# sgl-project/rbg

Hardware: NVIDIA B200
Metric: replica_x_node_affinity_scores_per_sec (higher is better)
Workload: dtype f32

## Files before the change

rbg_b200/csrc/kernels.cuh:

```cuda
#pragma once
#include <cuda_runtime.h>
#include <stdint.h>

#include "../../include/rbgtopo.h"

namespace rbgtopo {

constexpr int KS = RBGTOPO_MAX_STEP_REPLICAS;
constexpr int MAXP = RBGTOPO_MAX_STEP_ROLES;
constexpr int MAXQ = RBGTOPO_MAX_GROUP_ROLES;
constexpr int SCORE_THREADS = 256;
constexpr int SCORE_WARPS = SCORE_THREADS / 32;
constexpr int BASE_THREADS = 256;
constexpr int BASE_TILE_ROWS = 256;
constexpr int BASE_TILE_NNZ = 6144;
constexpr int FMIN_SMEM_MAX = 131072;
constexpr uint32_t FULL = 0xFFFFFFFFu;

struct TopoDev {
  int n;
  int slab_lo, slab_hi;
  int slab_stride;
  const int* row_ptr;
  const int* col;
// ... 23 lines not shown
  const int* perm;
  unsigned long long* lists;
  const unsigned long long* lists_all;
  long long part_stride;
  unsigned long long* merged;
  unsigned long long* excl;
  const unsigned long long* excl_all;
  long long excl_part_stride;
  int* dstar;
  int* assign;
  int* status;
  int* domain_out;
  int* corr;
  int* corr_cnt;
  int corr_w;
};

constexpr int EMIT_TAB_WORDS = 12;
__host__ __device__ __forceinline__ int emit_pack_role(int count, int demand, int need, int flags) {
  return count | (need << 6) | ((flags & RBGTOPO_ROLE_EXCLUSIVE) << 11) | (demand << 12);
}

__host__ __device__ __forceinline__ int emit_pack_row(int demand, int need, bool rexcl) {
  return need | ((rexcl ? 1 : 0) << 5) | (demand << 6);
}

__device__ __forceinline__ uint32_t orderable_u32(float x) {
  uint32_t b = __float_as_uint(x);
  return b ^ ((b >> 31) ? 0xFFFFFFFFu : 0x80000000u);
}
// ... 257 lines not shown
```

rbg_b200/csrc/plan_group.cuh:

```cuda
#pragma once
#include "select_fast.cuh"

namespace rbgtopo {

struct GroupTab {
  int* node;
  int* cons;
  float* aw;
  int mask, HT;
  int* cnt;
  int* dSlot;
  float* dBase;
  int* dFree;
  int* dAvail;
  int* dDom;
};
struct GroupRole {
  int count, demand, need, flags;
};

__host__ __device__ inline size_t group_smem_bytes(int QB, int PB, int HT, int CAP) {
  return (size_t)HT * 4 * (2 + QB) + (size_t)CAP * 20 +
         (size_t)PB * KS * (3 * 8 + 3 * 4) +
         (size_t)MAXP * 16 + (size_t)MAXP * RBGTOPO_MAX_GROUP_ROLES * 4;
// ... 215 lines not shown
      const bool rexcl = excl && (sR[wi][4 * ri + 3] & RBGTOPO_ROLE_EXCLUSIVE);
      sRec[wi][lane] = emit_pack_row(sR[wi][4 * ri + 2], max(0, min(need, RBGTOPO_NEED_CAP)), rexcl);
    }
    __syncwarp();
    for (int p = 0; p < P; ++p) {
      const int cnt = sCount[wi][p];
      const int2 rr = make_int2(sRec[wi][p], gid);
      if (lane < cnt && row + lane < n_rows) rtab[row + lane] = rr;
      row += cnt;
    }
    if (lane < P) sPl[wi][sRole[wi][lane]] += sCount[wi][lane];
    __syncwarp();
  }
}

template <bool DIRECT>
__global__ void __launch_bounds__(32 * MAXP, 4) k_plan_group(TopoDev t, BatchDev b, int QB, int HT, int CAP, int record) {
  extern __shared__ __align__(16) unsigned char pg_smem[];
  __shared__ int sTakenNode[KS], sTakenAmt[KS], sTakenRole[KS], sRowB[KS], sRowN[KS];
  __shared__ int sDstar, sCnt, sNew, sStatus, sAny, sCorrN;
  const int tid = threadIdx.x, warp = tid >> 5, lane = tid & 31, nthreads = blockDim.x, nwarps = nthreads >> 5;
  const int PB = nwarps;
  GroupTab T;
  T.node = reinterpret_cast<int*>(pg_smem);
  T.cons = T.node + HT;
  T.aw = reinterpret_cast<float*>(T.cons + HT);
  T.mask = HT - 1;
  T.HT = HT;
  T.cnt = &sCnt;
  T.dSlot = reinterpret_cast<int*>(T.aw + (size_t)QB * HT);
// ... 11 lines not shown
  float* sPair = reinterpret_cast<float*>(sRole + MAXP);

  if (record) pdl_launch_dependents();
  PCLK(30);
#ifdef RBGTOPO_PHASE_CLOCKS
  if (tid == 0 && blockIdx.x < 2048) { g_cta_ns[blockIdx.x * 4] = pg_gtime(); g_cta_ns[blockIdx.x * 4 + 3] = pg_smid(); }
#endif
  int wave_i = 0;
  int step = b.perm ? b.perm[blockIdx.x] : blockIdx.x;
  __shared__ int sGR[DIRECT ? 4 * RBGTOPO_MAX_GROUP_ROLES : 1];
  __shared__ int sGP[DIRECT ? RBGTOPO_MAX_GROUP_ROLES * RBGTOPO_MAX_GROUP_ROLES : 1];
  __shared__ int sPlaced[DIRECT ? RBGTOPO_MAX_GROUP_ROLES : 1];
  __shared__ int sWRole[DIRECT ? RBGTOPO_MAX_STEP_ROLES : 1], sWCount[DIRECT ? RBGTOPO_MAX_STEP_ROLES : 1];
  __shared__ int sWP, sWN, sCr, sTk;
  int g_rep0 = 0, g_pend = 0, g_i0 = 0, g_stat = 0, g_dom = -1;
  StepHdr h;
  if (DIRECT) {
    const int* rec = b.blob + RBGTOPO_HDR_WORDS + (size_t)step * RBGTOPO_GROUP_WORDS;
    h.gid = rec[0];
    h.flags = rec[1] & (RBGTOPO_STEP_EXCLUSIVE | RBGTOPO_STEP_GANG);
    h.fixed_domain = (rec[1] & RBGTOPO_STEP_EXCLUSIVE) ? rec[2] : -1;
    h.Q = rec[3];
    h.role_off = rec[4];
    h.pair_off = rec[5];
    h.n_anchors = rec[6];
    h.anchor_off = rec[7];
    h.i0 = 0;
    g_rep0 = rec[8];
    g_pend = rec[9];
    h.P = 0; h.R = 0; h.rep_off = g_rep0; h.rolerow_off = 0; h.next_step = 0; h.n_cons = 0; h.cons_off = 0;
  } else {
    h = load_hdr(b, step);
  }
  for (int i = tid; i < HT; i += nthreads) {
    T.node[i] = -1;
    T.cons[i] = 0;
  }
  for (int i = tid; i < QB * HT; i += nthreads) T.aw[i] = 0.0f;
  if (tid == 0) sCnt = 0;
  if (DIRECT) {
    for (int i = tid; i < 4 * h.Q; i += nthreads) sGR[i] = b.blob[h.role_off + i];
    for (int i = tid; i < h.Q * h.Q; i += nthreads) sGP[i] = b.blob[h.pair_off + i];
    if (tid < RBGTOPO_MAX_GROUP_ROLES) sPlaced[tid] = 0;
    if (tid == 0) { sCr = 0; sTk = 0; }
  }
  const bool excl_step = (h.flags & RBGTOPO_STEP_EXCLUSIVE) != 0;
  const bool gang = (h.flags & RBGTOPO_STEP_GANG) != 0;
  const int gid = h.gid, Q = h.Q;
  int fixed = excl_step ? h.fixed_domain : -1;
  g_dom = fixed;
  const size_t stride = (size_t)t.slab_stride;
  __syncthreads();

  {
    const int* anc = b.blob + h.anchor_off;
    for (int a = warp; a < h.n_anchors - h.i0; a += nwarps) gtab_add_anchor(t, T, anc[3 * a], anc[3 * a + 1], anc[3 * a + 2], 0);
  }
  int n_new = 0;
  int cnt_done = 0;

  while (true) {
    PCLK(wave_i * 8 + 0);
    const unsigned long long ob0 = lane < t.n ? t.order_all[lane] : 0ull;
    if (DIRECT) {
      if (tid == 0) {
        int cr = sCr, tk = sTk;
        const int P = wave_next(sGR, Q, cr, tk, sWRole, sWCount);
// ... 305 lines not shown
```

rbg_b200/csrc/rbgtopo.cu:

```cuda
#include <cuda_runtime.h>
#include <cub/device/device_radix_sort.cuh>
#include <nvtx3/nvToolsExt.h>

#include <algorithm>
#include <chrono>
#include <climits>
#include <cstdarg>
#include <cstdio>
#include <cstdlib>
#include <cstring>
#include <functional>
#include <memory>
#include <map>
#include <mutex>
#include <shared_mutex>
#include <string>
#include <vector>

#include "kernels.cuh"
#include "plan.cuh"
#include "score.cuh"
#include "emit_tma.cuh"
#include "emit_rows.cuh"
#include "select.cuh"
// ... 119 lines not shown
  long long patch_cap = 0;
  int max_cap = 0;
  std::vector<int> poff;
};

struct Batch {
  bool in_use = false;
  bool staged = false;
  bool ran = false;
  bool early_emit = false;
  bool d2h_enqueued = false;
  uint64_t epoch = 0;
  cudaStream_t stream = nullptr;
  cudaStream_t stream2 = nullptr;
  cudaEvent_t ev[8] = {};
  std::vector<cudaEvent_t> it_ev;
  int passes = 0, pend_launches = 0, untimed_or_timed_passes = 0;
  bool shard_timed = false;
  BatchMeta m;
  DevBuf<int> blob;
  DevBuf<float> matrix;
  DevBuf<unsigned long long> lists, merged, excl;
  DevBuf<int> cand;
  DevBuf<long long> emit_clk;
  DevBuf<int> etab, emit_ctr;
  DevBuf<int2> rtab;
  bool any_excl = false;
  int perm_n = 0;
  std::vector<char> pass_mid;
  const int32_t* prestaged_h = nullptr;
// ... 2 lines not shown
  bool tev = false;
  DevBuf<int> corr, corr_cnt;
  std::vector<int> wave_begin, wave_maxp;
  std::vector<int> step_group;
  std::vector<int> step_row;
  DevBuf<int> gsrc;
  long long aux_off = -1;
  int g_lo = 0;
  std::vector<int> grp_flags, grp_assign_off, grp_pending, grp_fixed;
  DevBuf<int> out;
  PinBuf<int> h_in, h_out;
  ~Batch() {
    if (stream) cudaStreamDestroy(stream);
    if (stream2) cudaStreamDestroy(stream2);
    for (auto& e : ev) if (e) cudaEventDestroy(e);
    for (auto& e : it_ev) cudaEventDestroy(e);
  }
};

}

struct rbgtopo_ctx {
  rbgtopo_config cfg{};
  int sm_count = 148;
  int slab_lo = 0, slab_hi = 0, slab_stride = 0, lc = 1, chunk = 2048;
  std::shared_mutex topo_mu;
  uint64_t topo_epoch = 0;
  std::mutex pool_mu;
  Topology topo;
  std::vector<std::unique_ptr<Batch>> batches;
  cudaStream_t ext_stream = nullptr;
  bool use_ext_stream = false;
  std::atomic<bool> kernel_timing{false};
  cudaStream_t topo_stream = nullptr;
  cudaEvent_t base_ready = nullptr;
  cudaEvent_t topo_ready = nullptr, ev_base_a = nullptr, ev_base_b = nullptr, fence_ev = nullptr;
  bool base_timing_pending = false;
  PinBuf<int> h_free[2], h_owner[2];
  cudaEvent_t stage_ev[2] = {nullptr, nullptr};
  unsigned stage_idx = 0;
  std::mutex stat_mu;
  DevBuf<unsigned long long> xbuf;
  DevBuf<int> p2p_ctr;
  P2PDev p2p{};
  int p2p_rows_cap = 0;
  bool p2p_ready = false;
  unsigned long long p2p_seq = 0;
  long long p2p_bytes_last = 0;
  std::vector<void*> p2p_opened;
  rbgtopo_timing last{};
  std::vector<float> last_score_ms, last_select_ms;
// ... 31 lines not shown
                          : (kEmitNoRegCap ? k_emit_tma<2, 1, false> : k_emit_tma<2, 4, false>);
}
const int kEmitBlockSteps =
    getenv("RBGTOPO_EMIT_BLOCK") ? std::min(EMIT_MAX_BLOCK, std::max(1, atoi(getenv("RBGTOPO_EMIT_BLOCK")))) : 4;
const int kSplitMinGroups =
    getenv("RBGTOPO_SPLIT_MIN_GROUPS") ? std::max(2, atoi(getenv("RBGTOPO_SPLIT_MIN_GROUPS"))) : (1 << 30);
const bool kCompactSortKey = getenv("RBGTOPO_WIDE_SORT_KEY") == nullptr;
const bool kRefreshGraph = getenv("RBGTOPO_NO_REFRESH_GRAPH") == nullptr;
const bool kSmallSort = getenv("RBGTOPO_SMALL_SORT") != nullptr;
const bool kVerifyPlan = getenv("RBGTOPO_VERIFY_PLAN") != nullptr;
const int kHostThreads = getenv("RBGTOPO_HOST_THREADS") ? std::max(1, atoi(getenv("RBGTOPO_HOST_THREADS"))) : 4;
const int kHostParallelMinGroups = getenv("RBGTOPO_HOST_PARALLEL_MIN") ? std::max(1, atoi(getenv("RBGTOPO_HOST_PARALLEL_MIN"))) : 4096;

inline bool timing_events(const rbgtopo_ctx* c) { return kProfileHost || c->kernel_timing.load(std::memory_order_relaxed); }

void compute_slab(rbgtopo_ctx* c, int n) {
  const int W = c->cfg.world, r = c->cfg.rank;
  auto bound = [&](int g) -> int {
    if (g <= 0) return 0;
    if (g >= W) return n;
    long long b = (long long)g * n / W;
    return (int)(b / 128 * 128);
  };
  c->slab_lo = bound(r);
  c->slab_hi = bound(r + 1);
  int max_len = 0;
  for (int g = 0; g < W; ++g) max_len = std::max(max_len, bound(g + 1) - bound(g));
  int tcfg = c->cfg.chunk_nodes > 0 ? c->cfg.chunk_nodes : 2048;
  tcfg = std::min(2048, std::max(128, round_up(tcfg, 128)));
  c->lc = std::max(1, (max_len + tcfg - 1) / tcfg);
// ... 95 lines not shown
  }
  return RBGTOPO_OK;
}

int enqueue_refresh(rbgtopo_ctx* c, cudaStream_t s, int part) {
  Topology& T = c->topo;
  if (part & 1) {
  k_prep<<<(T.n + 255) / 256, 256, 0, s>>>(T.n, T.free_.p, T.domain.p, T.owner.p, T.fmin.p,
                                           T.node_owner.p);
  const int fmin_bytes = round_up(T.n, 16);
  const int staged = T.n <= FMIN_SMEM_MAX ? 1 : 0;
  const size_t smem = (size_t)2 * (BASE_TILE_NNZ + 8) * 4 + (staged ? fmin_bytes : 0);
  const TopoDev td = topo_dev(c);
  k_base<<<T.n_tiles, BASE_THREADS, smem, s>>>(td, T.tiles.p, staged, fmin_bytes, T.base.p);
  }
  if (part == 3) CK(cudaEventRecord(c->base_ready, s));
  if (!(part & 2)) {
    CK(cudaGetLastError());
    return RBGTOPO_OK;
  }
  const TopoDev td = topo_dev(c);
  const int slab_len = c->slab_hi - c->slab_lo;
  auto p2_bytes = [](int n) { int p2 = 32; while (p2 < n) p2 <<= 1; return (size_t)p2 * 8; };
  if (slab_len > 0 && slab_len <= ORDER_SMALL_MAX && kSmallSort) {
    k_order_sort_small<<<1, ORDER_SMALL_THREADS, p2_bytes(slab_len), s>>>(T.base.p, c->slab_lo, c->slab_hi, T.order.p);
  } else if (slab_len > 0) {
    k_order_keys<<<(slab_len + 255) / 256, 256, 0, s>>>(td, c->slab_lo, c->slab_hi, T.key_nb, T.okeys.p);
    size_t tmp_bytes = T.sort_tmp.cap;
    CK(cub::DeviceRadixSort::SortKeysDescending(T.sort_tmp.p, tmp_bytes, T.okeys.p, T.order.p, slab_len, 0, T.key_bits, s));
    if (T.key_nb) k_order_expand<<<(slab_len + 255) / 256, 256, 0, s>>>(T.order.p, slab_len, T.key_nb);
  }
// ... 31 lines not shown
      if (g) cudaGraphDestroy(g);
      (void)cudaGetLastError();
    };
    capture(1, &T.refresh_exec);
    if (T.refresh_exec) capture(2, &T.order_exec);
    if (!T.order_exec && T.refresh_exec) {
      cudaGraphExecDestroy(T.refresh_exec);
      T.refresh_exec = nullptr;
    }
    T.refresh_ready = true;
  }
  const bool tev = timing_events(c);
  if (tev) CK(cudaEventRecord(c->ev_base_a, s));
  if (T.refresh_exec) {
    CK(cudaGraphLaunch(T.refresh_exec, s));
    CK(cudaEventRecord(c->base_ready, s));
    CK(cudaGraphLaunch(T.order_exec, s));
  } else {
    int rc = enqueue_refresh(c, s, 3);
    if (rc) return rc;
  }
  if (tev) CK(cudaEventRecord(c->ev_base_b, s));
  CK(cudaEventRecord(c->topo_ready, s));
  T.pos_valid = c->cfg.world == 1;
  c->base_timing_pending = tev;
  CK(cudaGetLastError());
  if (sync) {
    CK(cudaStreamSynchronize(s));
    harvest_base_ms(c);
  }
  std::lock_guard<std::mutex> g(c->stat_mu);
  c->launches += 3;
  return RBGTOPO_OK;
}

inline long long emit_items(int ns, int lc) {
  return (long long)((ns + kEmitBlockSteps - 1) / kEmitBlockSteps) * lc * kEmitBlockSteps;
}
// ... 107 lines not shown
  std::lock_guard<std::mutex> g(c->pool_mu);
  for (auto& b : c->batches)
    if (!b->in_use) {
      b->in_use = true;
      *out = b.get();
      return RBGTOPO_OK;
    }
  auto nb = std::make_unique<Batch>();
  CK(cudaStreamCreateWithFlags(&nb->stream, cudaStreamNonBlocking));
  {
    int lo = 0, hi = 0;
    CK(cudaDeviceGetStreamPriorityRange(&lo, &hi));
    CK(cudaStreamCreateWithPriority(&nb->stream2, cudaStreamNonBlocking, kSelectHighPriority ? hi : lo));
  }
  for (auto& e : nb->ev) CK(cudaEventCreate(&e));
  nb->in_use = true;
  *out = nb.get();
  c->batches.push_back(std::move(nb));
  return RBGTOPO_OK;
}
void release_batch(rbgtopo_ctx* c, Batch* b) {
  std::lock_guard<std::mutex> g(c->pool_mu);
  b->wave_begin.clear();
  b->d2h_enqueued = false;
  b->in_use = false;
  b->staged = false;
  b->ran = false;
}

cudaStream_t stream_of(rbgtopo_ctx* c, Batch* b) { return c->use_ext_stream ? c->ext_stream : b->stream; }
// ... 559 lines not shown
  if (cfg->device < 0 || cfg->device >= ndev) return fail(RBGTOPO_ENODEVICE, "device %d of %d", cfg->device, ndev);
  cudaDeviceProp prop;
  CK(cudaGetDeviceProperties(&prop, cfg->device));
  if (prop.major != 10)
    return fail(RBGTOPO_ENODEVICE, "device %d is sm_%d%d; kernels are built for sm_100a only", cfg->device,
                prop.major, prop.minor);
  CK(cudaSetDevice(cfg->device));
  auto c = std::make_unique<rbgtopo_ctx>();
  c->cfg = *cfg;
  c->cfg.emit_matrix = 1;
  c->sm_count = prop.multiProcessorCount;
  c->kernel_timing.store(kKernelTimingEnv);
  CK(cudaStreamCreateWithFlags(&c->topo_stream, cudaStreamNonBlocking));
  CK(cudaEventCreateWithFlags(&c->topo_ready, cudaEventDisableTiming));
  CK(cudaEventCreateWithFlags(&c->base_ready, cudaEventDisableTiming));
  CK(cudaFuncSetAttribute(k_order_sort_small, cudaFuncAttributeMaxDynamicSharedMemorySize, ORDER_SMALL_MAX * 8));
  CK(cudaEventCreate(&c->ev_base_a));
  CK(cudaEventCreate(&c->ev_base_b));
  CK(cudaEventCreateWithFlags(&c->fence_ev, cudaEventDisableTiming));
  for (auto& e : c->stage_ev) CK(cudaEventCreateWithFlags(&e, cudaEventDisableTiming));
  CK(cudaFuncSetAttribute(k_select_assign_fast, cudaFuncAttributeMaxDynamicSharedMemorySize, (int)kFastSmemMax));
  CK(cudaFuncSetAttribute(k_shard_select, cudaFuncAttributeMaxDynamicSharedMemorySize, (int)kFastSmemMax));
  CK(cudaFuncSetAttribute(k_plan_group<false>, cudaFuncAttributeMaxDynamicSharedMemorySize, (int)kFastSmemMax));
  CK(cudaFuncSetAttribute(k_plan_group<true>, cudaFuncAttributeMaxDynamicSharedMemorySize, (int)kFastSmemMax));
  CK(cudaFuncSetAttribute(k_plan_group<true>, cudaFuncAttributePreferredSharedMemoryCarveout, cudaSharedmemCarveoutMaxShared));
  CK(cudaFuncSetAttribute(emit_tma_fn(), cudaFuncAttributeMaxDynamicSharedMemorySize, (int)emit_tma_smem_bytes(kEmitStages)));
  CK(cudaFuncSetAttribute(emit_tma_fn(), cudaFuncAttributePreferredSharedMemoryCarveout, cudaSharedmemCarveoutMaxShared));
  CK(cudaFuncSetAttribute(k_plan_group<false>, cudaFuncAttributePreferredSharedMemoryCarveout, cudaSharedmemCarveoutMaxShared));
#ifdef RBGTOPO_PHASE_CLOCKS
  {
// ... 3 lines not shown
#endif
  *out = c.release();
  return RBGTOPO_OK;
}

int32_t rbgtopo_destroy(rbgtopo_ctx* c) {
  if (!c) return RBGTOPO_OK;
  cudaSetDevice(c->cfg.device);
  cudaDeviceSynchronize();
  for (void* q : c->p2p_opened) cudaIpcCloseMemHandle(q);
  if (c->topo.refresh_exec) cudaGraphExecDestroy(c->topo.refresh_exec);
  if (c->topo.order_exec) cudaGraphExecDestroy(c->topo.order_exec);
  if (c->topo_stream) cudaStreamDestroy(c->topo_stream);
  if (c->topo_ready) cudaEventDestroy(c->topo_ready);
  if (c->base_ready) cudaEventDestroy(c->base_ready);
  if (c->ev_base_a) cudaEventDestroy(c->ev_base_a);
  if (c->ev_base_b) cudaEventDestroy(c->ev_base_b);
  if (c->fence_ev) cudaEventDestroy(c->fence_ev);
  for (auto& e : c->stage_ev) if (e) cudaEventDestroy(e);
  delete c;
  return RBGTOPO_OK;
}

int32_t rbgtopo_set_topology(rbgtopo_ctx* c, int32_t n, int64_t e, const int32_t* row_ptr,
                             const int32_t* col, const int32_t* w, const int32_t* free_slots,
                             const int32_t* domain, int32_t n_domains, const int32_t* owner,
                             uint64_t generation) {
  if (!c || !row_ptr || !free_slots || !domain || !owner || (e > 0 && (!col || !w)))
    return fail(RBGTOPO_EINVAL, "null argument");
  if (n < 1 || e < 0 || e > 0x7FFFFFF0LL || n_domains < 1) return fail(RBGTOPO_EINVAL, "n=%d e=%lld", n, (long long)e);
// ... 180 lines not shown
  }
  CK(T.d_changed.reserve(2 * m));
  CK(cudaMemcpyAsync(T.d_changed.p, c->h_free[sb].p, 2 * m * 4, cudaMemcpyHostToDevice, s));
  CK(cudaEventRecord(c->stage_ev[sb], s));
  const bool incremental = c->cfg.world == 1 && T.pos_valid && est <= DELTA_MAX_AFFECTED && getenv("RBGTOPO_NO_DELTA") == nullptr;
  if (!incremental) {
    k_delta_scatter<<<(unsigned)((m + 255) / 256), 256, 0, s>>>(T.free_.p, T.d_changed.p, (int)m);
    CK(cudaGetLastError());
    return run_base(c, s, false);
  }
  const bool tev = timing_events(c);
  if (tev) CK(cudaEventRecord(c->ev_base_a, s));
  CK(cudaMemsetAsync(T.aff.p, 0, 4, s));
  const TopoDev td = topo_dev(c);
  k_delta_apply<<<(unsigned)((m * 32 + 255) / 256), 256, 0, s>>>(td, T.free_.p, T.fmin.p, T.base.p, T.d_changed.p, (int)m, T.flag.p, T.aff.p);
  CK(cudaEventRecord(c->base_ready, s));
  k_delta_sort<<<1, 1024, 0, s>>>(T.base.p, T.pos.p, T.flag.p, T.aff.p, T.new_keys.p, T.old_pos.p);
  const int n = c->slab_hi - c->slab_lo;
  k_delta_merge<<<(n + 255) / 256, 256, 0, s>>>(T.order.p, n, T.aff.p, T.new_keys.p, T.old_pos.p, T.order_alt.p, T.pos.p);
  CK(cudaMemcpyAsync(T.order.p, T.order_alt.p, (size_t)n * 8, cudaMemcpyDeviceToDevice, s));
  if (tev) CK(cudaEventRecord(c->ev_base_b, s));
  CK(cudaEventRecord(c->topo_ready, s));
  c->base_timing_pending = tev;
  CK(cudaGetLastError());
  std::lock_guard<std::mutex> g(c->stat_mu);
  c->launches += 3;
  return RBGTOPO_OK;
}

int32_t rbgtopo_score_assign(rbgtopo_ctx* c, const int32_t* blob, int64_t words, int32_t* assign,
                             int32_t* status, int32_t* domain) {
  if (!c) return fail(RBGTOPO_EINVAL, "null ctx");

  std::shared_lock<std::shared_mutex> lk(c->topo_mu);
  CK(cudaSetDevice(c->cfg.device));
  Batch* b = nullptr;
  int rc = acquire_batch(c, &b);
// ... 1079 lines not shown
  t.h2d_ms += b.h2d_ms;
  t.score_ms += b.score_ms;
  t.select_ms += b.select_ms;
  t.d2h_ms += b.d2h_ms;
  t.total_ms += b.total_ms;
  t.launches += b.launches;
  t.h2d_words += b.h2d_words;
  t.scores += b.scores;
  t.algo_bytes += b.algo_bytes;
  return t;
}
}

namespace {
const bool kNoDirect = getenv("RBGTOPO_NO_DIRECT") != nullptr;

struct GroupFacts {
  int pend = 0, nw = 0, max_p = 1, max_k = 1, i0_last = 0;
  long long pcp = 0;
};
struct ShapeFacts {
  bool valid = false;
  int q = 0, nw = 0, max_p = 1, max_k = 1, i0_last = 0;
  long long pend = 0;
  int32_t roles[4 * RBGTOPO_MAX_GROUP_ROLES];
  int32_t pair[RBGTOPO_MAX_GROUP_ROLES * RBGTOPO_MAX_GROUP_ROLES];
  long long role_bound[RBGTOPO_MAX_GROUP_ROLES];
  bool match(const int32_t* r, const int32_t* p, int qq) const {
    return valid && qq == q && memcmp(r, roles, (size_t)16 * qq) == 0 && memcmp(p, pair, (size_t)4 * qq * qq) == 0;
  }
// ... 132 lines not shown
  const int nb = 1024;
  static thread_local std::vector<int> bucket, wkey;
  bucket.assign(nb + 1, 0);
  wkey.resize((size_t)ng);
  for (int g = 0; g < ng; ++g) {
    if (facts[g].nw <= 0) continue;
    const long long w = (long long)facts[g].pend + std::max(0, gb[RBGTOPO_HDR_WORDS + (int64_t)g * RBGTOPO_GROUP_WORDS + 6]);
    wkey[g] = (nb - 1) - (int)(w * (nb - 1) / wmax);
    bucket[wkey[g] + 1] += 1;
  }
  for (int k = 0; k < nb; ++k) bucket[k + 1] += bucket[k];
  for (int g = 0; g < ng; ++g)
    if (facts[g].nw > 0) perm[bucket[wkey[g]]++] = g;
  return RBGTOPO_OK;
}
int direct_pass2(const TopoHost& th, const int32_t* gb, int64_t words, int ng, long long amax_limit, long long row_w,
                 std::vector<GroupFacts>& facts, DirectGeom* G) {
  int first_bad = ng;
#pragma omp parallel for schedule(static) num_threads(kHostThreads) reduction(min : first_bad) if (ng >= kHostParallelMinGroups && kHostThreads > 1)
  for (int g = 0; g < ng; ++g)
    if (group_facts(th, gb, words, g, false, amax_limit, row_w, &facts[g], 2) != RBGTOPO_OK) first_bad = std::min(first_bad, g);
  if (first_bad < ng) return group_facts(th, gb, words, first_bad, true, amax_limit, row_w, &facts[first_bad], 2);
  for (int g = 0; g < ng; ++g)
    if (facts[g].nw > 0)
      G->max_cap = std::max(G->max_cap, (long long)facts[g].i0_last + facts[g].pcp + (long long)facts[g].i0_last * th.max_degp1);
  G->nth = std::max(128, 32 * G->max_p);
  G->CAP = std::max(32, round_up((int)std::min<long long>(G->max_cap, 0x3FFFFFFF), 32));
  G->HT = 64;
  while (G->HT <= G->CAP && G->HT < (1 << 20)) G->HT <<= 1;
  G->smem = group_smem_bytes(G->max_q, G->nth / 32, G->HT, G->CAP);
// ... 12 lines not shown
  NvtxRange nv("rbgtopo:place_groups_direct");
  const Topology& T = c->topo;
  static const bool prof = kProfileHost;
  auto now = [] { return std::chrono::steady_clock::now(); };
  auto us = [](auto a, auto b2) { return std::chrono::duration<double, std::micro>(b2 - a).count(); };
  const auto t0 = now();
  Batch* b = nullptr;
  int rc = acquire_batch(c, &b);
  if (rc) return rc;
  cudaStream_t s = stream_of(c, b);
  auto done = [&](int r) {
    if (r || !*handled) cudaStreamSynchronize(s);
    release_batch(c, b);
    return r;
  };
  const size_t perm_off = ((size_t)words + 3) & ~(size_t)3;
  const size_t src_words = perm_off + (size_t)ng;
  bool rtab_early = false;
  rc = [&]() -> int {
    CK(b->h_in.reserve(src_words));
    CK(b->gsrc.reserve(src_words));
    b->tev = false;
    b->perm_n = 0;
    memcpy(b->h_in.p, gb, (size_t)words * 4);
    CK(cudaMemcpyAsync(b->gsrc.p, b->h_in.p, (size_t)words * 4, cudaMemcpyHostToDevice, s));
    if (gb[4] > 0 && (size_t)gb[4] <= b->rtab.cap) {
      k_group_rtab<<<(ng + RTAB_WARPS - 1) / RTAB_WARPS, 32 * RTAB_WARPS, 0, s>>>(b->gsrc.p, (int)words, ng, gb[4], b->rtab.p);
      rtab_early = true;
    }
    return RBGTOPO_OK;
  }();
  if (rc) return done(rc);
  const auto t1 = now();

  TopoHost th;
  th.n = T.n;
  th.n_domains = T.n_domains;
  th.degp1 = T.h_degp1.data();
  th.max_degp1 = T.max_degp1;
  th.wsum_max = T.wsum_max;
  const long long row_w = T.wsum_max + RBGTOPO_SELF_W;
  const long long amax_limit = ((1LL << 24) + row_w - 1) / row_w;
  static thread_local std::vector<GroupFacts> facts;
  DirectGeom G;
  rc = direct_pass1(th, gb, words, ng, amax_limit, row_w, facts, b->h_in.p + perm_off, &G);
  if (rc) return done(rc);
  const long long total_r = G.total_r;
  const int n0 = G.n0, max_q = G.max_q;
  const bool any_excl = G.any_excl;
  const long long segs = ((total_r + kEmitRowsBlock - 1) / kEmitRowsBlock) * c->lc;
  if (segs > 0x7FFFFFF0LL) return done(RBGTOPO_OK);
  const auto t2 = now();

  const size_t out_n = (size_t)total_r + 2 * (size_t)ng;
  rc = [&]() -> int {
    CK(b->matrix.reserve((size_t)std::max<long long>(1, total_r) * c->slab_stride));
    CK(b->rtab.reserve((size_t)std::max<long long>(1, total_r)));
    CK(b->out.reserve(out_n + 4));
    CK(b->h_out.reserve(out_n + 4));
    b->epoch = c->topo_epoch;
    if (n0 > 0) {
      CK(cudaMemcpyAsync(b->gsrc.p + perm_off, b->h_in.p + perm_off, (size_t)n0 * 4, cudaMemcpyHostToDevice, s));
      if (!rtab_early)
        k_group_rtab<<<(ng + RTAB_WARPS - 1) / RTAB_WARPS, 32 * RTAB_WARPS, 0, s>>>(b->gsrc.p, (int)words, ng, (int)total_r, b->rtab.p);
      CK(cudaStreamWaitEvent(s, c->base_ready, 0));
      CK(cudaStreamWaitEvent(s, c->topo_ready, 0));
      b->any_excl = any_excl;
      const int erc = launch_emit_plan(c, b, s, ng, total_r);
      if (erc) return erc;
    }
    return RBGTOPO_OK;
  }();
  if (rc) return done(rc);
  const auto t2b = now();

  rc = direct_pass2(th, gb, words, ng, amax_limit, row_w, facts, &G);
  if (rc) return done(rc);
  const int nth = G.nth, HT = G.HT, CAP = G.CAP;
  const size_t smem = G.smem;
  if (G.max_cap > 0x3FFFFFFFLL || smem > kFastSmemMax) return done(RBGTOPO_OK);
  const auto t2c = now();

  rc = [&]() -> int {
    if (n0 > 0) {
      BatchDev d{};
      d.blob = b->gsrc.p;
      d.n_steps = ng;
      d.lc = c->lc;
      d.chunk = c->chunk;
      d.parts = 1;
      d.matrix = b->matrix.p;
      d.assign = b->out.p;
      d.status = b->out.p + total_r;
      d.domain_out = d.status + ng;
      d.dstar = d.domain_out;
      d.perm = b->gsrc.p + perm_off;
      cudaLaunchConfig_t cfg{};
      cfg.gridDim = dim3((unsigned)n0);
      cfg.blockDim = dim3((unsigned)nth);
      cfg.dynamicSmemBytes = smem;
      cfg.stream = s;
      cudaLaunchAttribute at[1];
      at[0].id = cudaLaunchAttributeProgrammaticStreamSerialization;
      at[0].val.programmaticStreamSerializationAllowed = 1;
      cfg.attrs = at;
      cfg.numAttrs = kNoPdl ? 0 : 1;
      CK(cudaLaunchKernelEx(&cfg, k_plan_group<true>, topo_dev(c), d, (int)max_q, HT, CAP, 0));
      CK(cudaMemcpyAsync(b->h_out.p, b->out.p, out_n * 4, cudaMemcpyDeviceToHost, s));
    }
    const auto t3 = now();
    CK(cudaStreamSynchronize(s));
    CK(cudaGetLastError());
    const auto t4 = now();
    const int32_t* a = b->h_out.p;
    if (total_r > 0) memcpy(assign, a, (size_t)total_r * 4);
    if ((int)dirty->size() < ng) dirty->resize((size_t)ng, 0);
    for (int g = 0; g < ng; ++g) {
      const int32_t* rec = gb + RBGTOPO_HDR_WORDS + (int64_t)g * RBGTOPO_GROUP_WORDS;
      const bool excl = (rec[1] & RBGTOPO_STEP_EXCLUSIVE) != 0;
      int st = RBGTOPO_PLACED_ALL, dm = excl ? rec[2] : -1;
      if (facts[g].nw > 0) {
        st = a[total_r + g];
        dm = excl ? a[total_r + ng + g] : -1;
      }
      (*dirty)[g] = st == RBGTOPO_PLACED_PART;
      if (status) status[g] = st;
      if (domain) domain[g] = dm;
    }
    if (prof)
      fprintf(stderr, "[rbgtopo direct] stage %.0f us, pass 1 %.0f us, enqueue 1 %.0f us, pass 2 %.0f us, enqueue 2 %.0f us, wait %.0f us, results %.0f us\n",
              us(t0, t1), us(t1, t2), us(t2, t2b), us(t2b, t2c), us(t2c, t3), us(t3, t4), us(t4, now()));
    return RBGTOPO_OK;
  }();
  if (rc) return done(rc);
  {
    const long long slab = c->slab_hi - c->slab_lo;
    rbgtopo_timing tm{};
    tm.scores = total_r * slab;
    tm.algo_bytes = 4LL * total_r * slab + 4LL * words + 8LL * slab;
    tm.launches = n0 > 0 ? 3 : 0;
    tm.h2d_words = (int32_t)((long long)words + n0);
    std::lock_guard<std::mutex> g(c->stat_mu);
    c->last = tm;
    c->last_score_ms.clear();
    c->last_select_ms.clear();
    c->calls += 1;
    c->scores_total += tm.scores;
    c->launches += tm.launches;
  }
  *handled = true;
  return done(RBGTOPO_OK);
}

}

int32_t rbgtopo_place_groups(rbgtopo_ctx* c, const int32_t* gb, int64_t words, int32_t* assign,
                             int32_t* status, int32_t* domain) {
  if (!c || !gb || !assign) return fail(RBGTOPO_EINVAL, "null argument");
  std::vector<char> dirty;
  {
    std::shared_lock<std::shared_mutex> lk(c->topo_mu);
    if (!c->topo.valid) return fail(RBGTOPO_ENOTOPO, "set_topology has not been called");
    CK(cudaSetDevice(c->cfg.device));
// ... 129 lines not shown
  if (deg_plus1)
    for (int i = 0; i < n_nodes; ++i) {
      if (deg_plus1[i] < 1) return fail(RBGTOPO_EINVAL, "deg_plus1[%d]", i);
      th.max_degp1 = std::max(th.max_degp1, deg_plus1[i]);
    }
  th.wsum_max = wsum_max;
  const long long row_w = wsum_max + RBGTOPO_SELF_W;
  const long long amax_limit = ((1LL << 24) + row_w - 1) / row_w;
  static thread_local std::vector<GroupFacts> facts;
  static thread_local std::vector<int32_t> perm;
  perm.assign((size_t)std::max(1, ng), 0);
  DirectGeom G;
  int rc = direct_pass1(th, gb, words, ng, amax_limit, row_w, facts, perm.data(), &G);
  if (!rc) rc = direct_pass2(th, gb, words, ng, amax_limit, row_w, facts, &G);
  if (rc) return rc;
  geom[0] = (int32_t)G.total_r;
  geom[1] = G.n0;
  geom[2] = G.max_q;
  geom[3] = G.max_p;
  geom[4] = (int32_t)std::min<long long>(G.max_cap, 0x7FFFFFFF);
  geom[5] = G.nth;
  geom[6] = G.HT;
  geom[7] = G.CAP;
  if (order && order_cap > 0) memcpy(order, perm.data(), (size_t)std::min<int64_t>(order_cap, G.n0) * 4);
  return RBGTOPO_OK;
}

int32_t rbgtopo_stage_groups(rbgtopo_ctx* c, const int32_t* gb, int64_t words, int32_t* handle) {
  if (!c || !gb || !handle) return fail(RBGTOPO_EINVAL, "null argument");
  std::shared_lock<std::shared_mutex> lk(c->topo_mu);
// ... 526 lines not shown
```

Before: 1079 billion.

## Enqueue direct group select early with cached geometry, validating and retrying on device

The direct placement path now launches the emit and select kernels before host-side validation passes finish. It uses a quick host prescan for launch order and the geometry cached from the previous call, so GPU work overlaps the host validation. The kernel checks each group's header and capacity itself and marks a group for retry when the guessed geometry is too small; the host then relaunches those groups with the exact geometry. This adds in-kernel validation work and a possible second launch and sync, and it includes optional profiling events.

```diff
diff --git a/rbg_b200/csrc/kernels.cuh b/rbg_b200/csrc/kernels.cuh
--- a/rbg_b200/csrc/kernels.cuh
+++ b/rbg_b200/csrc/kernels.cuh
@@ -61,6 +61,7 @@
   int* corr;
   int* corr_cnt;
   int corr_w;
+  int words, n_rows, max_degp1;
 };
 
 constexpr int EMIT_TAB_WORDS = 12;
diff --git a/rbg_b200/csrc/plan_group.cuh b/rbg_b200/csrc/plan_group.cuh
--- a/rbg_b200/csrc/plan_group.cuh
+++ b/rbg_b200/csrc/plan_group.cuh
@@ -253,6 +253,8 @@
   }
 }
 
+constexpr int PG_RETRY = -100;
+
 template <bool DIRECT>
 __global__ void __launch_bounds__(32 * MAXP, 4) k_plan_group(TopoDev t, BatchDev b, int QB, int HT, int CAP, int record) {
   extern __shared__ __align__(16) unsigned char pg_smem[];
@@ -294,6 +296,9 @@
   __shared__ int sWRole[DIRECT ? RBGTOPO_MAX_STEP_ROLES : 1], sWCount[DIRECT ? RBGTOPO_MAX_STEP_ROLES : 1];
   __shared__ int sWP, sWN, sCr, sTk;
   int g_rep0 = 0, g_pend = 0, g_i0 = 0, g_stat = 0, g_dom = -1;
+  __shared__ int sChk;
+  __shared__ unsigned long long sPcpW[MAXP];
+  bool hdr_ok = true, bad = false;
   StepHdr h;
   if (DIRECT) {
     const int* rec = b.blob + RBGTOPO_HDR_WORDS + (size_t)step * RBGTOPO_GROUP_WORDS;
@@ -309,6 +314,12 @@
     g_rep0 = rec[8];
     g_pend = rec[9];
     h.P = 0; h.R = 0; h.rep_off = g_rep0; h.rolerow_off = 0; h.next_step = 0; h.n_cons = 0; h.cons_off = 0;
+    const long long W = b.words;
+    hdr_ok = h.Q >= 1 && h.Q <= min(QB, RBGTOPO_MAX_GROUP_ROLES) && h.role_off >= 0 && (long long)h.role_off + 4 * h.Q <= W &&
+             h.pair_off >= 0 && (long long)h.pair_off + h.Q * h.Q <= W && h.n_anchors >= 0 && h.anchor_off >= 0 &&
+             (long long)h.anchor_off + 3LL * h.n_anchors <= W && g_rep0 >= 0 && g_pend >= 1 &&
+             (long long)g_rep0 + g_pend <= b.n_rows;
+    bad = !hdr_ok;
   } else {
     h = load_hdr(b, step);
   }
@@ -319,8 +330,32 @@
   for (int i = tid; i < QB * HT; i += nthreads) T.aw[i] = 0.0f;
   if (tid == 0) sCnt = 0;
   if (DIRECT) {
-    for (int i = tid; i < 4 * h.Q; i += nthreads) sGR[i] = b.blob[h.role_off + i];
-    for (int i = tid; i < h.Q * h.Q; i += nthreads) sGP[i] = b.blob[h.pair_off + i];
+    unsigned long long pc = 0;
+    const int n_role_words = hdr_ok ? 4 * h.Q : 0, n_pair = hdr_ok ? h.Q * h.Q : 0, n_anc = hdr_ok ? h.n_anchors : 0;
+    for (int i = tid; i < n_role_words; i += nthreads) {
+      const int v = b.blob[h.role_off + i];
+      sGR[i] = v;
+      const int f = i & 3;
+      if (f == 0 && i >= 4 && v < b.blob[h.role_off + i - 4]) bad = true;
+      if ((f == 1 && (v < 0 || v > 0x3FFFFFFF)) || (f == 2 && (v < 0 || v > RBGTOPO_MAX_FREE))) bad = true;
+    }
+    for (int i = tid; i < n_pair; i += nthreads) {
+      const int v = b.blob[h.pair_off + i];
+      sGP[i] = v;
+      if (v < 0 || v > (1 << 24)) bad = true;
+    }
+    const int* anc = b.blob + h.anchor_off;
+    for (int a = tid; a < n_anc; a += nthreads) {
+      const int m = anc[3 * a], q = anc[3 * a + 1], c = anc[3 * a + 2];
+      if (m < 0 || m >= t.n || q < 0 || q >= h.Q || c < 0 || c > (1 << 24)) {
+        bad = true;
+        continue;
+      }
+      pc += (unsigned)(t.row_ptr[m + 1] - t.row_ptr[m] + 1);
+    }
+#pragma unroll
+    for (int o = 16; o > 0; o >>= 1) pc += __shfl_xor_sync(FULL, pc, o);
+    if (lane == 0) sPcpW[warp] = pc;
     if (tid < RBGTOPO_MAX_GROUP_ROLES) sPlaced[tid] = 0;
     if (tid == 0) { sCr = 0; sTk = 0; }
   }
@@ -330,7 +365,32 @@
   int fixed = excl_step ? h.fixed_domain : -1;
   g_dom = fixed;
   const size_t stride = (size_t)t.slab_stride;
-  __syncthreads();
+  const bool any_bad = __syncthreads_or(bad);
+  if (DIRECT) {
+    if (tid == 0) {
+      long long pend = 0, pcp = 0;
+      for (int i = 0; !any_bad && i < Q; ++i) pend += sGR[4 * i + 1];
+      for (int w = 0; w < nwarps; ++w) pcp += (long long)sPcpW[w];
+      bool ok = !any_bad && pend == g_pend;
+      int cr = 0, tk = 0, i0 = 0, i0_last = 0;
+      while (ok) {
+        const int P = wave_next(sGR, Q, cr, tk, sWRole, sWCount);
+        if (P == 0) break;
+        int n = 0;
+        for (int k = 0; k < P; ++k) n += sWCount[k];
+        ok = P <= nwarps;
+        i0_last = i0;
+        i0 += n;
+      }
+      ok = ok && (long long)i0_last + pcp + (long long)i0_last * b.max_degp1 <= CAP;
+      sChk = ok ? 0 : 1;
+    }
+    __syncthreads();
+    if (sChk) {
+      if (tid == 0) b.status[step] = PG_RETRY;
+      return;
+    }
+  }
 
   {
     const int* anc = b.blob + h.anchor_off;
diff --git a/rbg_b200/csrc/rbgtopo.cu b/rbg_b200/csrc/rbgtopo.cu
--- a/rbg_b200/csrc/rbgtopo.cu
+++ b/rbg_b200/csrc/rbgtopo.cu
@@ -157,6 +157,7 @@
   cudaStream_t stream = nullptr;
   cudaStream_t stream2 = nullptr;
   cudaEvent_t ev[8] = {};
+  cudaEvent_t pev[8] = {};
   std::vector<cudaEvent_t> it_ev;
   int passes = 0, pend_launches = 0, untimed_or_timed_passes = 0;
   bool shard_timed = false;
@@ -189,6 +190,7 @@
     if (stream) cudaStreamDestroy(stream);
     if (stream2) cudaStreamDestroy(stream2);
     for (auto& e : ev) if (e) cudaEventDestroy(e);
+    for (auto& e : pev) if (e) cudaEventDestroy(e);
     for (auto& e : it_ev) cudaEventDestroy(e);
   }
 };
@@ -210,6 +212,8 @@
   cudaStream_t topo_stream = nullptr;
   cudaEvent_t base_ready = nullptr;
   cudaEvent_t topo_ready = nullptr, ev_base_a = nullptr, ev_base_b = nullptr, fence_ev = nullptr;
+  cudaEvent_t prof_base = nullptr, prof_topo = nullptr;
+  struct { bool valid = false; int max_q = 1, nth = 128, HT = 64, CAP = 32; size_t smem = 0; } direct_geom;
   bool base_timing_pending = false;
   PinBuf<int> h_free[2], h_owner[2];
   cudaEvent_t stage_ev[2] = {nullptr, nullptr};
@@ -271,6 +275,12 @@
 
 inline bool timing_events(const rbgtopo_ctx* c) { return kProfileHost || c->kernel_timing.load(std::memory_order_relaxed); }
 
+cudaError_t record_ready(rbgtopo_ctx* c, cudaStream_t s, bool topo) {
+  cudaError_t e = cudaEventRecord(topo ? c->topo_ready : c->base_ready, s);
+  if (e == cudaSuccess && kProfileHost) e = cudaEventRecord(topo ? c->prof_topo : c->prof_base, s);
+  return e;
+}
+
 void compute_slab(rbgtopo_ctx* c, int n) {
   const int W = c->cfg.world, r = c->cfg.rank;
   auto bound = [&](int g) -> int {
@@ -396,7 +406,7 @@
   const TopoDev td = topo_dev(c);
   k_base<<<T.n_tiles, BASE_THREADS, smem, s>>>(td, T.tiles.p, staged, fmin_bytes, T.base.p);
   }
-  if (part == 3) CK(cudaEventRecord(c->base_ready, s));
+  if (part == 3) CK(record_ready(c, s, false));
   if (!(part & 2)) {
     CK(cudaGetLastError());
     return RBGTOPO_OK;
@@ -458,14 +468,14 @@
   if (tev) CK(cudaEventRecord(c->ev_base_a, s));
   if (T.refresh_exec) {
     CK(cudaGraphLaunch(T.refresh_exec, s));
-    CK(cudaEventRecord(c->base_ready, s));
+    CK(record_ready(c, s, false));
     CK(cudaGraphLaunch(T.order_exec, s));
   } else {
     int rc = enqueue_refresh(c, s, 3);
     if (rc) return rc;
   }
   if (tev) CK(cudaEventRecord(c->ev_base_b, s));
-  CK(cudaEventRecord(c->topo_ready, s));
+  CK(record_ready(c, s, true));
   T.pos_valid = c->cfg.world == 1;
   c->base_timing_pending = tev;
   CK(cudaGetLastError());
@@ -603,6 +613,8 @@
     CK(cudaStreamCreateWithPriority(&nb->stream2, cudaStreamNonBlocking, kSelectHighPriority ? hi : lo));
   }
   for (auto& e : nb->ev) CK(cudaEventCreate(&e));
+  if (kProfileHost)
+    for (auto& e : nb->pev) CK(cudaEventCreate(&e));
   nb->in_use = true;
   *out = nb.get();
   c->batches.push_back(std::move(nb));
@@ -1192,6 +1204,10 @@
   CK(cudaStreamCreateWithFlags(&c->topo_stream, cudaStreamNonBlocking));
   CK(cudaEventCreateWithFlags(&c->topo_ready, cudaEventDisableTiming));
   CK(cudaEventCreateWithFlags(&c->base_ready, cudaEventDisableTiming));
+  if (kProfileHost) {
+    CK(cudaEventCreate(&c->prof_base));
+    CK(cudaEventCreate(&c->prof_topo));
+  }
   CK(cudaFuncSetAttribute(k_order_sort_small, cudaFuncAttributeMaxDynamicSharedMemorySize, ORDER_SMALL_MAX * 8));
   CK(cudaEventCreate(&c->ev_base_a));
   CK(cudaEventCreate(&c->ev_base_b));
@@ -1225,6 +1241,8 @@
   if (c->topo_stream) cudaStreamDestroy(c->topo_stream);
   if (c->topo_ready) cudaEventDestroy(c->topo_ready);
   if (c->base_ready) cudaEventDestroy(c->base_ready);
+  if (c->prof_base) cudaEventDestroy(c->prof_base);
+  if (c->prof_topo) cudaEventDestroy(c->prof_topo);
   if (c->ev_base_a) cudaEventDestroy(c->ev_base_a);
   if (c->ev_base_b) cudaEventDestroy(c->ev_base_b);
   if (c->fence_ev) cudaEventDestroy(c->fence_ev);
@@ -1435,13 +1453,13 @@
   CK(cudaMemsetAsync(T.aff.p, 0, 4, s));
   const TopoDev td = topo_dev(c);
   k_delta_apply<<<(unsigned)((m * 32 + 255) / 256), 256, 0, s>>>(td, T.free_.p, T.fmin.p, T.base.p, T.d_changed.p, (int)m, T.flag.p, T.aff.p);
-  CK(cudaEventRecord(c->base_ready, s));
+  CK(record_ready(c, s, false));
   k_delta_sort<<<1, 1024, 0, s>>>(T.base.p, T.pos.p, T.flag.p, T.aff.p, T.new_keys.p, T.old_pos.p);
   const int n = c->slab_hi - c->slab_lo;
   k_delta_merge<<<(n + 255) / 256, 256, 0, s>>>(T.order.p, n, T.aff.p, T.new_keys.p, T.old_pos.p, T.order_alt.p, T.pos.p);
   CK(cudaMemcpyAsync(T.order.p, T.order_alt.p, (size_t)n * 8, cudaMemcpyDeviceToDevice, s));
   if (tev) CK(cudaEventRecord(c->ev_base_b, s));
-  CK(cudaEventRecord(c->topo_ready, s));
+  CK(record_ready(c, s, true));
   c->base_timing_pending = tev;
   CK(cudaGetLastError());
   std::lock_guard<std::mutex> g(c->stat_mu);
@@ -2551,6 +2569,15 @@
 
 namespace {
 const bool kNoDirect = getenv("RBGTOPO_NO_DIRECT") != nullptr;
+const bool kValidateFirst = getenv("RBGTOPO_VALIDATE_FIRST") != nullptr;
+enum TopoWait { kWaitEmit, kWaitSelect, kWaitAuto };
+const TopoWait kTopoWait = [] {
+  const char* v = getenv("RBGTOPO_TOPO_WAIT");
+  if (v && !strcmp(v, "emit")) return kWaitEmit;
+  if (v && !strcmp(v, "select")) return kWaitSelect;
+  return kWaitAuto;
+}();
+const bool kDirectRetryAll = getenv("RBGTOPO_DIRECT_RETRY_ALL") != nullptr;
 
 struct GroupFacts {
   int pend = 0, nw = 0, max_p = 1, max_k = 1, i0_last = 0;
@@ -2713,6 +2740,34 @@
     if (facts[g].nw > 0) perm[bucket[wkey[g]]++] = g;
   return RBGTOPO_OK;
 }
+int direct_prescan(const int32_t* gb, int ng, int32_t* perm, bool* any_excl) {
+  const int nb = 1024;
+  static thread_local std::vector<int> bucket, wkey;
+  bucket.assign(nb + 1, 0);
+  wkey.resize((size_t)ng);
+  long long wmax = 1;
+  *any_excl = false;
+  for (int g = 0; g < ng; ++g) {
+    const int32_t* rec = gb + RBGTOPO_HDR_WORDS + (int64_t)g * RBGTOPO_GROUP_WORDS;
+    if (rec[9] <= 0) continue;
+    wmax = std::max(wmax, (long long)rec[9] + std::max(0, rec[6]));
+    *any_excl |= (rec[1] & RBGTOPO_STEP_EXCLUSIVE) != 0;
+  }
+  int n0 = 0;
+  for (int g = 0; g < ng; ++g) {
+    const int32_t* rec = gb + RBGTOPO_HDR_WORDS + (int64_t)g * RBGTOPO_GROUP_WORDS;
+    if (rec[9] <= 0) continue;
+    const long long w = (long long)rec[9] + std::max(0, rec[6]);
+    wkey[g] = (nb - 1) - (int)(w * (nb - 1) / wmax);
+    bucket[wkey[g] + 1] += 1;
+    n0 += 1;
+  }
+  for (int k = 0; k < nb; ++k) bucket[k + 1] += bucket[k];
+  for (int g = 0; g < ng; ++g)
+    if (gb[RBGTOPO_HDR_WORDS + (int64_t)g * RBGTOPO_GROUP_WORDS + 9] > 0) perm[bucket[wkey[g]]++] = g;
+  return n0;
+}
+
 int direct_pass2(const TopoHost& th, const int32_t* gb, int64_t words, int ng, long long amax_limit, long long row_w,
                  std::vector<GroupFacts>& facts, DirectGeom* G) {
   int first_bad = ng;
@@ -2755,19 +2810,96 @@
     release_batch(c, b);
     return r;
   };
+  const bool pev = prof && b->pev[0];
+  auto mark = [&](int i) { return pev ? cudaEventRecord(b->pev[i], s) : cudaSuccess; };
   const size_t perm_off = ((size_t)words + 3) & ~(size_t)3;
   const size_t src_words = perm_off + (size_t)ng;
+  const long long rows0 = gb[4];
+  const size_t out_n0 = (size_t)std::max(0LL, rows0) + 2 * (size_t)ng;
+  decltype(c->direct_geom) guess;
+  {
+    std::lock_guard<std::mutex> g(c->stat_mu);
+    guess = c->direct_geom;
+  }
+  if (kDirectRetryAll && guess.valid) {
+    guess.max_q = 0;
+    guess.nth = 128;
+    guess.HT = 64;
+    guess.CAP = 32;
+    guess.smem = group_smem_bytes(0, 4, 64, 32);
+  }
+  const bool early = !kValidateFirst && guess.valid && rows0 > 0 && (size_t)rows0 <= b->rtab.cap &&
+                     (size_t)rows0 * c->slab_stride <= b->matrix.cap && out_n0 + 4 <= b->out.cap && out_n0 + 4 <= b->h_out.cap &&
+                     ((rows0 + kEmitRowsBlock - 1) / kEmitRowsBlock) * c->lc <= 0x7FFFFFF0LL;
   bool rtab_early = false;
+  int n0_early = 0;
+  auto select_dev = [&](int grid, const int32_t* perm_d, int qb, int nth, int HT, int CAP, size_t smem, bool pdl,
+                        long long n_rows) -> int {
+    BatchDev d{};
+    d.blob = b->gsrc.p;
+    d.n_steps = ng;
+    d.lc = c->lc;
+    d.chunk = c->chunk;
+    d.parts = 1;
+    d.matrix = b->matrix.p;
+    d.assign = b->out.p;
+    d.status = b->out.p + n_rows;
+    d.domain_out = d.status + ng;
+    d.dstar = d.domain_out;
+    d.perm = perm_d;
+    d.words = (int)words;
+    d.n_rows = (int)n_rows;
+    d.max_degp1 = T.max_degp1;
+    cudaLaunchConfig_t cfg{};
+    cfg.gridDim = dim3((unsigned)grid);
+    cfg.blockDim = dim3((unsigned)nth);
+    cfg.dynamicSmemBytes = smem;
+    cfg.stream = s;
+    cudaLaunchAttribute at[1];
+    at[0].id = cudaLaunchAttributeProgrammaticStreamSerialization;
+    at[0].val.programmaticStreamSerializationAllowed = 1;
+    cfg.attrs = at;
+    cfg.numAttrs = pdl && !kNoPdl ? 1 : 0;
+    CK(cudaLaunchKernelEx(&cfg, k_plan_group<true>, topo_dev(c), d, qb, HT, CAP, 0));
+    return RBGTOPO_OK;
+  };
   rc = [&]() -> int {
     CK(b->h_in.reserve(src_words));
     CK(b->gsrc.reserve(src_words));
     b->tev = false;
     b->perm_n = 0;
     memcpy(b->h_in.p, gb, (size_t)words * 4);
+    CK(mark(0));
     CK(cudaMemcpyAsync(b->gsrc.p, b->h_in.p, (size_t)words * 4, cudaMemcpyHostToDevice, s));
+    CK(mark(1));
     if (gb[4] > 0 && (size_t)gb[4] <= b->rtab.cap) {
       k_group_rtab<<<(ng + RTAB_WARPS - 1) / RTAB_WARPS, 32 * RTAB_WARPS, 0, s>>>(b->gsrc.p, (int)words, ng, gb[4], b->rtab.p);
       rtab_early = true;
+    }
+    CK(mark(2));
+    if (!early) return RBGTOPO_OK;
+    bool any_excl = false;
+    n0_early = direct_prescan(gb, ng, b->h_in.p + perm_off, &any_excl);
+    if (n0_early > 0) {
+      CK(cudaMemcpyAsync(b->gsrc.p + perm_off, b->h_in.p + perm_off, (size_t)n0_early * 4, cudaMemcpyHostToDevice, s));
+      CK(cudaStreamWaitEvent(s, c->base_ready, 0));
+      if (kTopoWait == kWaitEmit) CK(cudaStreamWaitEvent(s, c->topo_ready, 0));
+      b->any_excl = any_excl;
+      CK(mark(3));
+      const int erc = launch_emit_plan(c, b, s, ng, rows0);
+      if (erc) return erc;
+      CK(mark(4));
+      bool pdl = true;
+      if (kTopoWait == kWaitSelect || (kTopoWait == kWaitAuto && cudaEventQuery(c->topo_ready) != cudaSuccess)) {
+        CK(cudaStreamWaitEvent(s, c->topo_ready, 0));
+        pdl = false;
+      }
+      (void)cudaGetLastError();
+      const int src = select_dev(n0_early, b->gsrc.p + perm_off, guess.max_q, guess.nth, guess.HT, guess.CAP, guess.smem, pdl, rows0);
+      if (src) return src;
+      CK(mark(5));
+      CK(cudaMemcpyAsync(b->h_out.p, b->out.p, out_n0 * 4, cudaMemcpyDeviceToHost, s));
+      CK(mark(6));
     }
     return RBGTOPO_OK;
   }();
@@ -2783,23 +2915,28 @@
   const long long row_w = T.wsum_max + RBGTOPO_SELF_W;
   const long long amax_limit = ((1LL << 24) + row_w - 1) / row_w;
   static thread_local std::vector<GroupFacts> facts;
+  static thread_local std::vector<int32_t> perm1;
+  perm1.resize((size_t)ng);
+  int32_t* perm = early ? perm1.data() : b->h_in.p + perm_off;
   DirectGeom G;
-  rc = direct_pass1(th, gb, words, ng, amax_limit, row_w, facts, b->h_in.p + perm_off, &G);
+  rc = direct_pass1(th, gb, words, ng, amax_limit, row_w, facts, perm, &G);
   if (rc) return done(rc);
   const long long total_r = G.total_r;
   const int n0 = G.n0, max_q = G.max_q;
   const bool any_excl = G.any_excl;
   const long long segs = ((total_r + kEmitRowsBlock - 1) / kEmitRowsBlock) * c->lc;
   if (segs > 0x7FFFFFF0LL) return done(RBGTOPO_OK);
+  if (early && (n0 != n0_early || total_r != rows0))
+    return done(fail(RBGTOPO_EINVAL, "internal: pre-scan of the groups blob disagrees with its validation"));
   const auto t2 = now();
 
   const size_t out_n = (size_t)total_r + 2 * (size_t)ng;
   rc = [&]() -> int {
+    if (early) return RBGTOPO_OK;
     CK(b->matrix.reserve((size_t)std::max<long long>(1, total_r) * c->slab_stride));
     CK(b->rtab.reserve((size_t)std::max<long long>(1, total_r)));
     CK(b->out.reserve(out_n + 4));
     CK(b->h_out.reserve(out_n + 4));
-    b->epoch = c->topo_epoch;
     if (n0 > 0) {
       CK(cudaMemcpyAsync(b->gsrc.p + perm_off, b->h_in.p + perm_off, (size_t)n0 * 4, cudaMemcpyHostToDevice, s));
       if (!rtab_early)
@@ -2807,12 +2944,15 @@
       CK(cudaStreamWaitEvent(s, c->base_ready, 0));
       CK(cudaStreamWaitEvent(s, c->topo_ready, 0));
       b->any_excl = any_excl;
+      CK(mark(3));
       const int erc = launch_emit_plan(c, b, s, ng, total_r);
       if (erc) return erc;
+      CK(mark(4));
     }
     return RBGTOPO_OK;
   }();
   if (rc) return done(rc);
+  b->epoch = c->topo_epoch;
   const auto t2b = now();
 
   rc = direct_pass2(th, gb, words, ng, amax_limit, row_w, facts, &G);
@@ -2823,37 +2963,33 @@
   const auto t2c = now();
 
   rc = [&]() -> int {
-    if (n0 > 0) {
-      BatchDev d{};
-      d.blob = b->gsrc.p;
-      d.n_steps = ng;
-      d.lc = c->lc;
-      d.chunk = c->chunk;
-      d.parts = 1;
-      d.matrix = b->matrix.p;
-      d.assign = b->out.p;
-      d.status = b->out.p + total_r;
-      d.domain_out = d.status + ng;
-      d.dstar = d.domain_out;
-      d.perm = b->gsrc.p + perm_off;
-      cudaLaunchConfig_t cfg{};
-      cfg.gridDim = dim3((unsigned)n0);
-      cfg.blockDim = dim3((unsigned)nth);
-      cfg.dynamicSmemBytes = smem;
-      cfg.stream = s;
-      cudaLaunchAttribute at[1];
-      at[0].id = cudaLaunchAttributeProgrammaticStreamSerialization;
-      at[0].val.programmaticStreamSerializationAllowed = 1;
-      cfg.attrs = at;
-      cfg.numAttrs = kNoPdl ? 0 : 1;
-      CK(cudaLaunchKernelEx(&cfg, k_plan_group<true>, topo_dev(c), d, (int)max_q, HT, CAP, 0));
+    if (n0 > 0 && !early) {
+      const int src = select_dev(n0, b->gsrc.p + perm_off, max_q, nth, HT, CAP, smem, true, total_r);
+      if (src) return src;
+      CK(mark(5));
       CK(cudaMemcpyAsync(b->h_out.p, b->out.p, out_n * 4, cudaMemcpyDeviceToHost, s));
+      CK(mark(6));
     }
     const auto t3 = now();
     CK(cudaStreamSynchronize(s));
     CK(cudaGetLastError());
     const auto t4 = now();
-    const int32_t* a = b->h_out.p;
+    int n_retry = 0;
+    int32_t* const a = b->h_out.p;
+    int32_t* const rl = b->h_in.p + perm_off;
+    for (int g = 0; g < ng; ++g)
+      if (facts[g].nw > 0 && a[total_r + g] == PG_RETRY) rl[n_retry++] = g;
+    if (n_retry > 0) {
+      CK(cudaMemcpyAsync(b->gsrc.p + perm_off, rl, (size_t)n_retry * 4, cudaMemcpyHostToDevice, s));
+      const int src = select_dev(n_retry, b->gsrc.p + perm_off, max_q, nth, HT, CAP, smem, false, total_r);
+      if (src) return src;
+      CK(cudaMemcpyAsync(b->h_out.p, b->out.p, out_n * 4, cudaMemcpyDeviceToHost, s));
+      CK(cudaStreamSynchronize(s));
+      CK(cudaGetLastError());
+      for (int g = 0; g < ng; ++g)
+        if (facts[g].nw > 0 && a[total_r + g] == PG_RETRY) return fail(RBGTOPO_EINVAL, "internal: group %d does not fit its exact launch geometry", g);
+    }
+    const auto t5 = now();
     if (total_r > 0) memcpy(assign, a, (size_t)total_r * 4);
     if ((int)dirty->size() < ng) dirty->resize((size_t)ng, 0);
     for (int g = 0; g < ng; ++g) {
@@ -2868,9 +3004,22 @@
       if (status) status[g] = st;
       if (domain) domain[g] = dm;
     }
-    if (prof)
-      fprintf(stderr, "[rbgtopo direct] stage %.0f us, pass 1 %.0f us, enqueue 1 %.0f us, pass 2 %.0f us, enqueue 2 %.0f us, wait %.0f us, results %.0f us\n",
-              us(t0, t1), us(t1, t2), us(t2, t2b), us(t2b, t2c), us(t2c, t3), us(t3, t4), us(t4, now()));
+    if (prof) {
+      fprintf(stderr, "[rbgtopo direct] %s, stage %.0f us, pass 1 %.0f us, enqueue 1 %.0f us, pass 2 %.0f us, enqueue 2 %.0f us, "
+                      "wait %.0f us, retry %d groups %.0f us, results %.0f us\n",
+              early ? "enqueue first" : "validate first", us(t0, t1), us(t1, t2), us(t2, t2b), us(t2b, t2c), us(t2c, t3), us(t3, t4),
+              n_retry, us(t4, t5), us(t5, now()));
+      if (pev && n0 > 0) {
+        auto dev = [&](cudaEvent_t e) {
+          float ms = 0.f;
+          return cudaEventElapsedTime(&ms, b->pev[0], e) == cudaSuccess ? ms * 1e3 : -1e9;
+        };
+        fprintf(stderr, "[rbgtopo direct] device: base_ready %.0f topo_ready %.0f upload %.0f rtab %.0f emit %.0f-%.0f select %.0f d2h %.0f us\n",
+                dev(c->prof_base), dev(c->prof_topo), dev(b->pev[1]), dev(b->pev[2]), dev(b->pev[3]), dev(b->pev[4]), dev(b->pev[5]),
+                dev(b->pev[6]));
+        (void)cudaGetLastError();
+      }
+    }
     return RBGTOPO_OK;
   }();
   if (rc) return done(rc);
@@ -2888,6 +3037,12 @@
     c->calls += 1;
     c->scores_total += tm.scores;
     c->launches += tm.launches;
+    c->direct_geom.valid = true;
+    c->direct_geom.max_q = max_q;
+    c->direct_geom.nth = nth;
+    c->direct_geom.HT = HT;
+    c->direct_geom.CAP = CAP;
+    c->direct_geom.smem = smem;
   }
   *handled = true;
   return done(RBGTOPO_OK);
@@ -3047,6 +3202,12 @@
   int rc = direct_pass1(th, gb, words, ng, amax_limit, row_w, facts, perm.data(), &G);
   if (!rc) rc = direct_pass2(th, gb, words, ng, amax_limit, row_w, facts, &G);
   if (rc) return rc;
+  static thread_local std::vector<int32_t> perm_pre;
+  perm_pre.assign(perm.size(), 0);
+  bool excl_pre = false;
+  const int n0_pre = direct_prescan(gb, ng, perm_pre.data(), &excl_pre);
+  if (n0_pre != G.n0 || excl_pre != G.any_excl || memcmp(perm_pre.data(), perm.data(), (size_t)G.n0 * 4) != 0)
+    return fail(RBGTOPO_EINVAL, "internal: the pre-scan's launch order differs from pass 1's");
   geom[0] = (int32_t)G.total_r;
   geom[1] = G.n0;
   geom[2] = G.max_q;
```

Result: no change. 1083 billion, median of 6 (+0.4%).
